# Shamir-Lab/Faucet

Measured on AMD Instinct MI355X. Metric: canonical k-mers/s (load+scan) at k=31, 100bp reads; % HBM roofline, higher is better.
Workload: dtype u64

## Files before the change

### faucet_amd/build.py

```python
from __future__ import annotations

import glob
import os
import subprocess
import sys

HERE = os.path.dirname(os.path.abspath(__file__))
ROOT = os.path.dirname(HERE)
CSRC = os.path.join(HERE, "csrc")
LIB = os.path.join(HERE, "libfaucet_gpu.so")
CLI = os.path.join(HERE, "faucet")
HIP_SOURCES = ["api.hip", "pack.hip", "load.hip", "load_slices.hip", "estimate.hip", "scan_pure.hip", "scan_walk.hip", "scan_table.hip", "scan_harvest.hip", "diag.hip", "text.hip", "stage3.hip", "stage3_emit.hip", "stage3_join.hip", "pairs.hip", "group.hip"]
CPP_SOURCES = ["sizing.cpp", "raw_plan.cpp", "tips_plan.cpp"]
HEADERS = ["fgpu_ctx.h", "fgpu_device.h", "fgpu_flags.h", "load_common.h", "walk_tables.h", "stage3_bits.h", "build_graph.h", os.path.join(ROOT, "include", "faucet_gpu.h")]
HIPCC = os.environ.get("HIPCC", "/opt/rocm/bin/hipcc")
FLAGS = ["-O3", "-std=c++17", "--offload-arch=gfx950", "-fPIC", "-Wall", "-Wno-unused-function", "-Wno-unused-result", "-Wno-unused-value"] + os.environ.get("FGPU_EXTRA_CXXFLAGS", "").split()


def _newer(target, deps):
    if not os.path.exists(target):
        return True
    t = os.path.getmtime(target)
    return any(os.path.getmtime(d) > t for d in deps)


def _run(cmd):
    r = subprocess.run(cmd, capture_output=True, text=True)
    if r.returncode != 0:
        sys.stderr.write(" ".join(cmd) + "\n" + r.stdout + r.stderr)
        raise RuntimeError("build failed: " + os.path.basename(cmd[-1]))
    if r.stderr.strip():
        sys.stderr.write(r.stderr)


def build(force: bool = False, jobs: int = 6) -> str:
    objdir = os.path.join(HERE, "build")
    os.makedirs(objdir, exist_ok=True)
    hdrs = [h if os.path.isabs(h) else os.path.join(CSRC, h) for h in HEADERS]
    objs, procs = [], []
    for src in HIP_SOURCES + CPP_SOURCES:
        sp = os.path.join(CSRC, src)
        obj = os.path.join(objdir, src + ".o")
        objs.append(obj)
        if force or _newer(obj, [sp] + hdrs):
            cmd = [HIPCC] + FLAGS + (["-x", "hip"] if src.endswith(".hip") else []) + ["-c", sp, "-o", obj]
            procs.append((cmd, subprocess.Popen(cmd, stdout=subprocess.PIPE, stderr=subprocess.STDOUT, text=True)))
            if len(procs) >= jobs:
# ... 28 lines not shown
```

### faucet_amd/csrc/fgpu_ctx.h

```cpp
#pragma once
#include <chrono>
#include <hip/hip_runtime.h>
#include <stdint.h>
#include <stdio.h>
#include <string.h>

#include <string>
#include <thread>
#include <vector>

#include "../../include/faucet_gpu.h"
#include <deque>

#include "fgpu_device.h"

#define FGPU_PADW 8
#define FGPU_USUAL_SPAN (1ULL << 26)
#define FGPU_MAX_SPAN (1ULL << 26)

#define FGPU_RANGE_EVENTS 16
#define FGPU_RANGE_MIN (1ULL << 20)

struct DevBuf {
    void*    p = nullptr;
// ... 486 lines not shown
int fgpu_stage_pack(fgpu_ctx* ctx, const fgpu_reads* reads);
int fgpu_stage_pack_block(fgpu_ctx* ctx, const fgpu_reads* reads, PackedBlock** out);
int fgpu_packed_acquire(fgpu_ctx* ctx, uint64_t T, uint64_t n_reads, int state, const char* who, PackedBlock** out, uint64_t beside = 0);
int fgpu_offs_keep(fgpu_ctx* ctx, void* dst, const uint64_t* src, uint64_t n);
int fgpu_offs_check_report(fgpu_ctx* ctx);
int fgpu_packed_digest(fgpu_ctx* ctx, const PackedBlock* b, bool verify);
int fgpu_host_batch_done(fgpu_ctx* ctx, const fgpu_reads* reads);
int fgpu_stage_load(fgpu_ctx* ctx, const void* codes, const void* bad, uint64_t T, uint64_t n_words);
int fgpu_resident_keep(fgpu_ctx* ctx);
int fgpu_resident_adopt(fgpu_ctx* ctx, const PackedBlock& b, const fgpu_kept_reads* reads = nullptr);
void fgpu_adopted_release(fgpu_ctx* ctx, std::vector<void*>* blocks);
int fgpu_stage_pack_keep(fgpu_ctx* ctx, const fgpu_reads* reads, uint64_t budget_left, PackedBlock* out, bool* no_memory);
void fgpu_estimate_drop_kept(fgpu_ctx* ctx);
int fgpu_load_sweep(fgpu_ctx* ctx);
int fgpu_stage_fixup(fgpu_ctx* ctx, const uint32_t* prefix);
int fgpu_stage_presence(fgpu_ctx* ctx);
int fgpu_epoch_before_batch(fgpu_ctx* ctx, uint64_t span);
int fgpu_epoch_after_batch(fgpu_ctx* ctx, uint64_t span);
enum { FGPU_TAKE_OK = 0, FGPU_TAKE_NO_BUDGET, FGPU_TAKE_NO_MEMORY };
int fgpu_resident_take(fgpu_ctx* ctx, const uint64_t (&parts)[5], bool budgeted, ResidentBatch** out, uint64_t* total);
int fgpu_pull_counters(fgpu_ctx* ctx);
int fgpu_check_reads(fgpu_ctx* ctx, const fgpu_reads* r);
void fgpu_load_pass_policy(fgpu_ctx* ctx);
int fgpu_load_pass_counters(fgpu_ctx* ctx);
int fgpu_load_pass_end(fgpu_ctx* ctx, fgpu_load_stats* stats);
int fgpu_load_pair_begin(fgpu_ctx* ctx);
int fgpu_load_pair_end(fgpu_ctx* ctx);
void fgpu_resident_reset(fgpu_ctx* ctx, bool keep_going);
int fgpu_stage_scan_pure(fgpu_ctx* ctx, uint64_t* n_pieces, bool one_range);
bool fgpu_walk_no_overlap();
int fgpu_stage_scan_walk(fgpu_ctx* ctx, uint64_t n_pieces);
int fgpu_stage_scan_need(fgpu_ctx* ctx);
int fgpu_stage_scan_need_lookup(fgpu_ctx* ctx, uint64_t w_lo, uint64_t w_hi);
int fgpu_stage_scan_need_prewalk(fgpu_ctx* ctx, uint64_t w_lo, uint64_t w_hi);
int fgpu_scan_refresh_planes(fgpu_ctx* ctx, BatchBufs* b);
int fgpu_scan_build_cand(fgpu_ctx* ctx, BatchBufs* b);
int fgpu_scan_import_probe(fgpu_ctx* ctx, const void* dev_entries, uint64_t n, uint64_t after_seq, uint32_t* dfilter, uint64_t dfilter_bits,
                           uint64_t* max_seq, uint64_t* n_newer, uint64_t digest[2]);
int fgpu_stage_scan_debug_drop(fgpu_ctx* ctx, uint64_t w_lo, uint64_t w_hi);
int fgpu_estimate_range_counts(fgpu_ctx* ctx, uint64_t g0, uint64_t g1, uint64_t h[2 * FGPU_EST_LEVELS + 1]);
void fgpu_estimate_close(fgpu_ctx* ctx, void** later);
int fgpu_estimate_finish(fgpu_ctx* ctx, fgpu_estimate* e, const char* who);
int fgpu_util_count_segments(fgpu_ctx* ctx, const void* bad, uint64_t n_words, int minlen);
int fgpu_util_popcount(fgpu_ctx* ctx, const void* dev, uint64_t nbytes, unsigned long long* dev_out);
int fgpu_util_or(fgpu_ctx* ctx, void* dst, const void* src, uint64_t nbytes);
int fgpu_util_probe_hash(fgpu_ctx* ctx, const uint64_t* d_kmers, uint64_t n, uint64_t* d_canon, uint64_t* d_hA, uint64_t* d_hB);
int fgpu_util_probe_contains(fgpu_ctx* ctx, const uint32_t* bloom, const uint64_t* d_canon, uint64_t n, unsigned char* d_out);
int fgpu_util_probe_stage3(fgpu_ctx* ctx, const uint64_t* d_kmers, uint64_t n, int mode, signed char* d_out);
int fgpu_scan_alloc(fgpu_ctx* ctx);
int fgpu_scan_harvest(fgpu_ctx* ctx, BatchBufs* b);
int fgpu_long_pairs_batch(fgpu_ctx* ctx, const fgpu_stop* d_stops, uint64_t n_stops, uint64_t n_reads);
int fgpu_long_pairs_reset(fgpu_ctx* ctx);
int fgpu_long_pairs_close(fgpu_ctx* ctx);
int fgpu_place_pair(fgpu_ctx* ctx);
int fgpu_scan_reset(fgpu_ctx* ctx);
int fgpu_scan_grow(fgpu_ctx* ctx, uint64_t new_cap);
int fgpu_scan_reserve(fgpu_ctx* ctx, uint64_t records);
int fgpu_scan_clear_table(fgpu_ctx* ctx);
int fgpu_scan_dump_order_impl(fgpu_ctx* ctx, const uint64_t* d_keys, const uint64_t* counts, const uint64_t* buckets, uint64_t n_phases, uint64_t n, uint32_t* order_host);
int fgpu_scan_regrow_empty(fgpu_ctx* ctx, uint64_t new_cap);
```

### faucet_amd/csrc/fgpu_device.h

```cpp
#pragma once
#include <hip/hip_runtime.h>
#include <stdint.h>

#define FD_SEED0 0xffaa54ffe6e6e6e7ULL
#define FD_SEED1 0x1140aada557088a4ULL

struct FdParams {
    int      k;
    int      j;
    int      n_hash;
    int      max_spacer;
    uint64_t kmask;
    uint64_t tai_mask;
};

__device__ __forceinline__ uint64_t fd_revcomp(uint64_t x, int k) {
    uint64_t y = __builtin_bitreverse64(x ^ 0xAAAAAAAAAAAAAAAAULL);
    y = ((y >> 1) & 0x5555555555555555ULL) | ((y & 0x5555555555555555ULL) << 1);
    return y >> (64 - 2 * k);
}

__device__ __forceinline__ uint64_t fd_canon(uint64_t x, int k) {
    uint64_t r = fd_revcomp(x, k);
    return x < r ? x : r;
// ... 61 lines not shown
__device__ __forceinline__ bool fd_bloom_contains_canon_lazy(const uint32_t* __restrict__ bloom, uint64_t canon,
                                                             uint64_t tai_mask, int n_hash) {
    const uint64_t hA = fd_old_hash(canon, FD_SEED0) & tai_mask;
    if (!((bloom[hA >> 5] >> (hA & 31)) & 1u)) return false;
    if (n_hash == 1) return true;
    const uint64_t hB = fd_old_hash(canon, FD_SEED1) & tai_mask;
    uint64_t h = (hA + hB) & tai_mask;
    for (int i = 1; i < n_hash; i++) {
        if (!((bloom[h >> 5] >> (h & 31)) & 1u)) return false;
        h = (h + hB) & tai_mask;
    }
    return true;
}

__device__ __forceinline__ void fd_bloom_set(uint32_t* bloom, uint64_t hA, uint64_t hB, uint64_t tai_mask, int n_hash) {
    uint64_t h = hA;
    for (int i = 0; i < n_hash; i++) {
        uint32_t bit = 1u << (h & 31);
        if (!(bloom[h >> 5] & bit)) atomicOr(&bloom[h >> 5], bit);
        h = (h + hB) & tai_mask;
    }
}

__device__ __forceinline__ uint64_t fd_mix(uint64_t x) {
    x ^= x >> 33;
    x *= 0xff51afd7ed558ccdULL;
    x ^= x >> 33;
    x *= 0xc4ceb9fe1a85ec53ULL;
    x ^= x >> 33;
    return x;
}

__device__ __forceinline__ int fd_lane() { return (int)(threadIdx.x & 63); }

__device__ __forceinline__ void wave_add(unsigned long long* dst, unsigned long long v) {
    for (int o = 32; o > 0; o >>= 1) v += __shfl_down(v, o, 64);
    if (fd_lane() == 0 && v) atomicAdd(dst, v);
}

__device__ __forceinline__ void block_add(unsigned long long* dst, unsigned long long v) {
    __shared__ unsigned long long part[4];
    for (int o = 32; o > 0; o >>= 1) v += __shfl_down(v, o, 64);
    if (fd_lane() == 0) part[threadIdx.x >> 6] = v;
    __syncthreads();
    if (threadIdx.x == 0) {
        const unsigned long long t = part[0] + part[1] + part[2] + part[3];
        if (t) atomicAdd(dst, t);
    }
    __syncthreads();
}
```

### faucet_amd/csrc/scan_pure.hip

```cpp
#include <algorithm>

#include "fgpu_ctx.h"
#include "fgpu_flags.h"

namespace {

__global__ void __launch_bounds__(256) k_scan_same(const uint64_t* __restrict__ codes, const uint64_t* __restrict__ kept_codes, uint64_t n_code_words,
                                                   const uint64_t* __restrict__ bad, const uint64_t* __restrict__ kept_bad, uint64_t n_words,
                                                   uint32_t* same) {
    bool differ = false;
    for (uint64_t i = (uint64_t)blockIdx.x * blockDim.x + threadIdx.x; i < n_code_words; i += (uint64_t)gridDim.x * blockDim.x) {
        differ |= codes[i] != kept_codes[i];
        if (i < n_words) differ |= bad[i] != kept_bad[i];
    }
    if (__ballot(differ) && fd_lane() == 0) *same = 0;
}

__global__ void __launch_bounds__(256) k_scan_valid(const uint64_t* __restrict__ codes, const uint64_t* __restrict__ bad,
                                                    uint64_t T, uint64_t n_words, FdParams fp, const uint32_t* __restrict__ bloom,
                                                    const uint64_t* __restrict__ sure, const uint32_t* __restrict__ same,
                                                    uint64_t* __restrict__ valid, DevCounters* cnt) {
    unsigned long long n_ok = 0, n_reused = 0;
    const uint64_t total = n_words * 64;
    const bool reuse = sure && *same != 0;
    for (uint64_t p = (uint64_t)blockIdx.x * blockDim.x + threadIdx.x; p < total; p += (uint64_t)gridDim.x * blockDim.x) {
        bool ok = p < T && fd_window_ok(bad, p, fp.k);
        bool v = false;
        if (ok) {
            n_ok++;
            if (reuse && ((sure[p >> 6] >> (p & 63)) & 1ULL)) {
                v = true;
                n_reused++;
            } else {
                v = fd_bloom_contains_canon(bloom, fd_canon(fd_kmer_at(codes, p, fp.k), fp.k), fp.tai_mask, fp.n_hash);
            }
        }
        uint64_t vm = __ballot(v);
        if (fd_lane() == 0) valid[p >> 6] = vm;
    }
    block_add(&cnt->kmers, n_ok);
    block_add(&cnt->valid_reused, n_reused);
}

__global__ void __launch_bounds__(256) k_scan_pieces(const uint64_t* __restrict__ valid, const uint64_t* __restrict__ bad,
                                                     uint64_t n_words, FdParams fp, int check_segment,
                                                     unsigned long long* pm, uint64_t* __restrict__ ps, DevCounters* cnt) {
    unsigned long long n_pieces = 0;
    for (uint64_t w = (uint64_t)blockIdx.x * blockDim.x + threadIdx.x; w < n_words; w += (uint64_t)gridDim.x * blockDim.x) {
        uint64_t vw = valid[w];
        uint64_t prev = w ? valid[w - 1] >> 63 : 0;
        uint64_t starts = vw & ~((vw << 1) | prev);
// ... 118 lines not shown
    while (lo < hi) {
        const uint64_t mid = (lo + hi + 1) >> 1;
        if ((offs[mid] - off0) + mid <= s0) lo = mid; else hi = mid - 1;
    }
    piece_read[i] = (uint32_t)lo;
}

__global__ void __launch_bounds__(256) k_scan_flags(const uint64_t* __restrict__ codes, const uint64_t* __restrict__ pm,
                                                    const uint64_t* __restrict__ need, uint64_t T, uint64_t w_lo, uint64_t w_hi, FdParams fp, const uint32_t* __restrict__ bloom,
                                                    unsigned long long* ff, unsigned long long* fb, unsigned long long* cf0,
                                                    unsigned long long* cf1, unsigned long long* cb0, unsigned long long* cb1,
                                                    DevCounters* cnt) {
    const int lane = fd_lane();
    const uint64_t n_waves = ((uint64_t)gridDim.x * blockDim.x) >> 6;
    const uint64_t n_chunks = (w_hi - w_lo + 3) / 4;
    unsigned long long n_eval = 0, n_piece = 0;
    for (uint64_t chunk = ((uint64_t)blockIdx.x * blockDim.x + threadIdx.x) >> 6; chunk < n_chunks; chunk += n_waves) {
        uint64_t mine = 0;
        if (lane < 8) {
            const uint64_t w = w_lo + chunk * 4 + (lane & 3);
            if (w < w_hi) {
                const uint64_t tmask = (w + 1) * 64 <= T ? ~0ULL : (T > w * 64 ? (1ULL << (T - w * 64)) - 1 : 0ULL);
                const uint64_t pmw = pm[w] & tmask, nd = need[w] & tmask;
                if (lane < 4) {
                    mine = nd & pmw & ((pmw >> 1) | (pm[w + 1] << 63));
                    n_eval += __popcll(nd);
                    n_piece += __popcll(pmw);
                } else {
                    mine = nd & pmw & ((pmw << 1) | (w ? pm[w - 1] >> 63 : 0ULL));
                }
            }
        }
        uint64_t m[8];
        int cum[9];
        cum[0] = 0;
#pragma unroll
        for (int q = 0; q < 8; q++) {
            m[q] = __shfl(mine, q, 64);
            cum[q + 1] = cum[q] + __popcll(m[q]);
        }
        for (int t = lane; t < cum[8]; t += 64) {
            int q = 0;
            uint64_t mq = m[0];
            int before = 0;
#pragma unroll
            for (int c = 1; c < 8; c++)
                if (t >= cum[c]) { q = c; mq = m[c]; before = cum[c]; }
            const int bit = select_bit(mq, t - before);
            const uint64_t w = w_lo + chunk * 4 + (q & 3);
            const uint64_t pos = w * 64 + bit;
            const uint64_t km = fd_kmer_at(codes, pos, fp.k);
            bool flag;
            int njc;
            const unsigned long long bm = 1ULL << bit;
            if (q < 4) {
                test_for_junction(km, fd_base_at(codes, pos + fp.k), fp, bloom, flag, njc);
                if (flag) atomicOr(&ff[w], bm);
                if (njc & 1) atomicOr(&cf0[w], bm);
                if (njc & 2) atomicOr(&cf1[w], bm);
            } else {
                test_for_junction(fd_revcomp(km, fp.k), fd_base_at(codes, pos - 1) ^ 2, fp, bloom, flag, njc);
                if (flag) atomicOr(&fb[w], bm);
                if (njc & 1) atomicOr(&cb0[w], bm);
                if (njc & 2) atomicOr(&cb1[w], bm);
            }
        }
    }
    block_add(&cnt->flag_positions, n_eval);
    block_add(&cnt->piece_positions, n_piece);
}

struct FlagPool {
    unsigned long long mf[64], mb[64];
    int excl[64];
};

struct FlagChain {
    uint64_t key;
    uint64_t hA, hB;
    uint32_t w;
    uint32_t st;
// ... 281 lines not shown
    BatchBufs& bb = *ctx->cur;
    *n_pieces = 0;
    bb.n_pieces = 0;
    bb.n_ranges = 0;
    if (bb.T == 0) return FGPU_OK;
    const uint64_t wb = (bb.n_words + FGPU_PADW) * 8;
    int rc;
    DevBuf* planes[] = {&bb.valid, &bb.pm, &bb.ps, &bb.ff, &bb.fb, &bb.cf0, &bb.cf1, &bb.cb0, &bb.cb1, &bb.inF, &bb.inB, &bb.lk, &bb.nF, &bb.nB, &bb.need};
    for (DevBuf* b : planes)
        if ((rc = fgpu_ensure_b(ctx, b, wb))) return rc;
    if ((rc = fgpu_ensure_b(ctx, &bb.ps_prefix, (bb.n_words + FGPU_PADW + bb.n_words / SCAN_BLOCK + 2) * 4))) return rc;
    const double t_a = fgpu_host_now();
    FGPU_HIP(hipMemsetAsync(bb.valid.p, 0, wb, ctx->stream));
    FGPU_HIP(hipMemsetAsync(bb.pm.p, 0, wb, ctx->stream));
    FGPU_HIP(hipMemsetAsync(bb.ps.p, 0, wb, ctx->stream));

    const unsigned grid = fgpu_grid(bb.n_words * 64, 256);
    const unsigned wgrid = fgpu_grid(bb.n_words, 256);
    if ((rc = fgpu_util_count_segments(ctx, ctx->cur->bad.p, ctx->cur->n_words, ctx->fd.k + 2 * ctx->fd.j + 1))) return rc;
    const uint64_t kept_index = ctx->scan_resident_base + ctx->scan_batch_index;
    const ResidentBatch* kept = kept_index < ctx->resident_count ? ctx->resident[kept_index] : nullptr;
    ctx->scan_batch_index++;
    if (kept && (kept->T != bb.T || kept->n_words != bb.n_words)) kept = nullptr;
    const bool taken = ctx->scan_take_kept != nullptr;
    if (taken) kept = ctx->scan_take_kept;
    if (kept) {
        if ((rc = fgpu_ensure_b(ctx, &bb.same, 64))) return rc;
        FGPU_HIP(hipMemsetAsync(bb.same.p, 0x01, 4, ctx->stream));
        const uint64_t ncw = 2 * bb.n_words;
        if (!taken)
            FGPU_LAUNCH("scan_same", k_scan_same, fgpu_grid(ncw, 256), 256, (const uint64_t*)bb.codes.p, (const uint64_t*)kept->codes_p(), ncw,
                        (const uint64_t*)bb.bad.p, (const uint64_t*)kept->bad_p(), bb.n_words, (uint32_t*)bb.same.p);
    }
    FGPU_LAUNCH("scan_valid", k_scan_valid, grid, 256, (const uint64_t*)bb.codes.p, (const uint64_t*)bb.bad.p, bb.T, bb.n_words, ctx->fd,
                (const uint32_t*)ctx->bloo2, kept ? (const uint64_t*)kept->sure.p : (const uint64_t*)nullptr,
                kept ? (const uint32_t*)bb.same.p : (const uint32_t*)nullptr, (uint64_t*)bb.valid.p, ctx->counters);
    const int check_segment = ctx->fd.k < 2 * ctx->fd.j + 2;
    FGPU_LAUNCH("scan_pieces", k_scan_pieces, wgrid, 256, (const uint64_t*)bb.valid.p, (const uint64_t*)bb.bad.p, bb.n_words, ctx->fd,
                check_segment, (unsigned long long*)bb.pm.p, (uint64_t*)bb.ps.p, ctx->counters);
    uint32_t* prefix = (uint32_t*)bb.ps_prefix.p;
    uint32_t* block_sums = prefix + bb.n_words + FGPU_PADW;
    const uint32_t nblk = fgpu_blocks(bb.n_words + 1, SCAN_BLOCK);
    const uint64_t nw1 = bb.n_words + 1;
    FGPU_LAUNCH("prefix_block", k_prefix_block, nblk, SCAN_BLOCK, (const uint64_t*)bb.ps.p, nw1, prefix, block_sums);
    FGPU_LAUNCH("prefix_sums", k_prefix_sums, 1, SCAN_BLOCK, block_sums, nblk);
    FGPU_LAUNCH("prefix_apply", k_prefix_apply, fgpu_blocks(nw1, 256), 256, prefix, (const uint32_t*)block_sums, nw1);
    FGPU_HIP(hipMemcpyAsync(ctx->counters_host, ctx->counters, sizeof(DevCounters), hipMemcpyDeviceToHost, ctx->stream));
    const double t_b = fgpu_host_now();
    FGPU_HIP(fgpu_sync_stream(ctx, ctx->stream));
    const double t_c = fgpu_host_now();
    ctx->host_ms[2] += t_b - t_a;
    ctx->host_ms[3] += t_c - t_b;
    bb.max_piece_span = ctx->counters_host->max_read_len + 64;
    const uint64_t np = ctx->counters_host->pieces - ctx->scan_pieces_seen;
    ctx->scan_pieces_seen = ctx->counters_host->pieces;
    *n_pieces = np;
    bb.n_pieces = np;
    if ((rc = fgpu_ensure_b(ctx, &bb.pieces, (np + 1) * sizeof(uint2)))) return rc;
    if (np) {
        FGPU_LAUNCH("piece_list", k_scan_piece_list, wgrid, 256, (const uint64_t*)bb.ps.p, (const uint64_t*)bb.pm.p,
                    (const uint32_t*)prefix, bb.n_words, (uint2*)bb.pieces.p);
        if (ctx->record_stops) {
            if ((rc = fgpu_ensure_b(ctx, &bb.piece_read, np * 4))) return rc;
            FGPU_LAUNCH("piece_read", k_scan_piece_read, fgpu_blocks(np, 256), 256, (const uint2*)bb.pieces.p, np, bb.d_offs, bb.n_reads,
                        (uint32_t*)bb.piece_read.p);
        }
        if ((rc = fgpu_stage_scan_need(ctx))) return rc;
        DevBuf* outs[] = {&bb.ff, &bb.fb, &bb.cf0, &bb.cf1, &bb.cb0, &bb.cb1};
        for (DevBuf* o : outs) FGPU_HIP(hipMemsetAsync(o->p, 0, wb, ctx->stream));
// ... 6 lines not shown
```

### faucet_amd/csrc/scan_walk.hip

```cpp
#include <cstring>
#include <algorithm>

#include "fgpu_flags.h"
#include "walk_tables.h"

namespace {

__device__ __forceinline__ uint32_t uf_find(uint32_t* parent, uint32_t x) {
    uint32_t p = ld_agent(&parent[x]);
    while (p != x) {
        uint32_t gp = ld_agent(&parent[p]);
        if (gp != p) atomicMin(&parent[x], gp);
        x = p;
        p = gp;
    }
    return x;
}

__device__ __forceinline__ void uf_union(uint32_t* parent, uint32_t a, uint32_t b) {
    for (;;) {
        a = uf_find(parent, a);
        b = uf_find(parent, b);
        if (a == b) return;
        if (a < b) { uint32_t t = a; a = b; b = t; }
        uint32_t old = atomicCAS(&parent[a], a, b);
        if (old == a) return;
    }
}

constexpr int W_OWNER_BITS = 24;
constexpr uint64_t W_OWNER_MASK = (1ULL << W_OWNER_BITS) - 1;
constexpr uint64_t W_EPOCH_MASK = 0xFFULL << 56;
constexpr uint32_t W_NO_OWNER = (uint32_t)W_OWNER_MASK;
__device__ __forceinline__ uint32_t wt_filter_bit(const WTable& wt, uint32_t h32) { return (h32 * 0x85EBCA6Bu) >> wt.fshift; }

__device__ __forceinline__ void wt_register(const WTable& wt, uint32_t* parent, uint32_t h32, uint32_t piece, DevCounters* cnt) {
// ... 75 lines not shown
    const WinDesc wd = make_window(pl, lo, hi);
    if (blockIdx.x < word_blocks) {
        const uint64_t w = (wd.lo >> 6) + (uint64_t)blockIdx.x * blockDim.x + threadIdx.x;
        if (w * 64 >= pos_end) return;
        unsigned long long m = pl.pm[w] & (pl.inF[w] | pl.inB[w] | pl.ff[w] | pl.fb[w]);
        if (w == (wd.lo >> 6)) m &= ~0ULL << (wd.lo & 63);
        if ((w + 1) * 64 > pos_end) m &= (1ULL << (pos_end & 63)) - 1;
        while (m) {
            const int b = __builtin_ctzll(m);
            m &= m - 1;
            const uint64_t p = w * 64 + (uint64_t)b;
            uint32_t li;
            uint2 pc;
            if (piece_in_window(pl, wd, p, li, pc)) wt_register(wt, parent, pl.kh[p], li, cnt);
        }
    } else if (blockIdx.x < word_blocks + piece_blocks) {
        const uint32_t li = (blockIdx.x - word_blocks) * blockDim.x + threadIdx.x;
        if (li >= wd.n) return;
        const uint2 pc = pl.pieces[wd.first_piece + li];
        const uint32_t len = pc.y + (uint32_t)fp.k - 1;
        wt_register(wt, parent, pl.kh[pc.x + (len / 2 - (uint32_t)fp.k / 2)], li, cnt);
        for (uint32_t q = (uint32_t)fp.max_spacer - 1; q < pc.y; q++) wt_register(wt, parent, pl.kh[pc.x + q], li, cnt);
    } else {
        const uint64_t t = (uint64_t)(blockIdx.x - word_blocks - piece_blocks) * blockDim.x + threadIdx.x;
        const uint64_t stride = (uint64_t)(gridDim.x - word_blocks - piece_blocks) * blockDim.x;
        for (int r = 0; r < FGPU_DELTA_RING; r++) {
            if (!ds.list[r]) continue;
            const uint64_t n = *ds.count[r];
            for (uint64_t i = t; i < n; i += stride) wt_register(wt, nullptr, ds.list[r][i], W_NO_OWNER, cnt);
        }
    }
}

__global__ void __launch_bounds__(256) k_walk_link(Planes pl, FdParams fp, WTable wt, uint32_t* parent, uint64_t lo, uint64_t hi,
                                                   uint64_t pos_end, uint32_t* roots_state) {
    const WinDesc wd = make_window(pl, lo, hi);
    if (roots_state && blockIdx.x == 0 && threadIdx.x == 0) { roots_state[0] = 0; roots_state[1] = 0; }
    const uint64_t base0 = wd.lo & ~63ULL;
    constexpr int U = 4;
    for (uint64_t base = base0 + (uint64_t)blockIdx.x * (256 * U); base < pos_end; base += (uint64_t)gridDim.x * (256 * U)) {
        uint64_t p[U];
        uint32_t h[U], fw[U];
        bool act[U];
#pragma unroll
        for (int u = 0; u < U; u++) {
            p[u] = base + (uint64_t)u * 256 + threadIdx.x;
            act[u] = p[u] >= wd.lo && p[u] < pos_end && ((pl.pm[p[u] >> 6] >> (p[u] & 63)) & 1ULL);
        }
#pragma unroll
        for (int u = 0; u < U; u++) h[u] = act[u] ? pl.kh[p[u]] : 0u;
#pragma unroll
        for (int u = 0; u < U; u++) {
            const uint32_t b = wt_filter_bit(wt, h[u]);
            fw[u] = act[u] ? ((wt.bits[b >> 5] >> (b & 31)) & 1u) : 0u;
        }
#pragma unroll
        for (int u = 0; u < U; u++) {
            bool hit = false;
            if (fw[u]) {
                uint64_t slot = 0;
                uint32_t owner = wt_owner(wt, h[u], slot);
                if (owner != U_INF) {
                    uint32_t li;
                    uint2 pc;
                    if (piece_in_window(pl, wd, p[u], li, pc)) {
                        hit = true;
                        if (owner == W_NO_OWNER) {
// ... 2075 lines not shown
    WTable wt;
    uint32_t *roots_state, *root_list;
};

struct LargeClusterRule {
    uint32_t ko_heavy;
    uint32_t ko_heavy_w;
    int ovw_rounds;
    bool ovw_on;
};

constexpr int OVW_MARK_LOG2 = 22;

template <class FullPass>
static int walk_dbg_compare(fgpu_ctx* ctx, hipStream_t st, const uint64_t* plane0, const uint64_t* plane1, uint64_t n_words, FullPass full, const char* what,
                            uint64_t batch, uint64_t lo) {
    uint64_t* scratch = nullptr;
    unsigned long long* out = nullptr;
    FGPU_HIP(hipMalloc(&scratch, 2 * n_words * 8));
    FGPU_HIP(hipMalloc(&out, 32));
    FGPU_HIP(hipMemsetAsync(out, 0, 32, st));
    FGPU_HIP(full(scratch));
    hipLaunchKernelGGL(k_dbg_diff, dim3(64), dim3(256), 0, st, (const uint64_t*)scratch, plane0, n_words, out, 0);
    if (plane1) hipLaunchKernelGGL(k_dbg_diff, dim3(64), dim3(256), 0, st, (const uint64_t*)(scratch + n_words), plane1, n_words, out, 1);
    unsigned long long h[4] = {0, 0, 0, 0};
    FGPU_HIP(hipMemcpyAsync(h, out, 32, hipMemcpyDeviceToHost, st));
    FGPU_HIP(hipStreamSynchronize(st));
    ctx->refresh_mismatch += h[0] + h[1];
    if (h[0] + h[1]) fprintf(stderr, "[fgpu] %s: %llu + %llu words differ, batch %llu window at %llu\n", what, h[0], h[1], (unsigned long long)batch, (unsigned long long)lo);
    (void)hipFree(scratch); (void)hipFree(out);
    return FGPU_OK;
}

static int walk_refresh_prepared(fgpu_ctx* ctx, BatchBufs& bb, const JTable& jt, hipStream_t walk_stream, bool* cand_ok) {
    *cand_ok = false;
    if (!(ctx->delta_ready && bb.planes_gen == ctx->hint_gen)) {
        FGPU_LAUNCH("walk_lookup", k_refresh_lookup, fgpu_grid(bb.n_words * 64, 256), 256, (const uint64_t*)bb.codes.p, (const uint64_t*)bb.pm.p, bb.n_words,
                    ctx->fd, jt, (const uint32_t*)jt.filter, jt.filter_mask, (uint64_t*)bb.nF.p, (uint64_t*)bb.nB.p, (const uint32_t*)bb.kh.p, 0, (uint64_t*)nullptr);
        ctx->refresh_full++;
        return FGPU_OK;
    }
    *cand_ok = !ctx->no_sparse_link && bb.cand.p && bb.cand_gen == ctx->hint_gen;
    if (ctx->delta_keys || ctx->refresh_delta)
        FGPU_LAUNCH("walk_lookup", k_refresh_lookup, fgpu_grid(bb.n_words * 64, 256), 256, (const uint64_t*)bb.codes.p, (const uint64_t*)bb.pm.p, bb.n_words,
                    ctx->fd, jt, (const uint32_t*)ctx->delta_filter.p, ctx->delta_filter_bits - 1, (uint64_t*)bb.nF.p, (uint64_t*)bb.nB.p,
                    (const uint32_t*)bb.kh.p, 1, *cand_ok ? (uint64_t*)bb.cand.p : (uint64_t*)nullptr);
    ctx->refresh_delta++;
    if (!ctx->dbg_delta_check) return FGPU_OK;
    const auto full = [&](uint64_t* scratch) {
        hipLaunchKernelGGL(k_refresh_lookup, dim3(fgpu_grid(bb.n_words * 64, 256)), dim3(256), 0, walk_stream, (const uint64_t*)bb.codes.p, (const uint64_t*)bb.pm.p,
                           bb.n_words, ctx->fd, jt, (const uint32_t*)jt.filter, jt.filter_mask, scratch, scratch + bb.n_words, (const uint32_t*)bb.kh.p, 0,
                           (uint64_t*)nullptr);
        return hipSuccess;
    };
    return walk_dbg_compare(ctx, walk_stream, (const uint64_t*)bb.nF.p, (const uint64_t*)bb.nB.p, bb.n_words, full, "merged in-map planes against planes made again",
                            bb.seq, 0);
}

static int walk_wait_range(fgpu_ctx* ctx, const WalkBatch& wb, uint64_t pos_end) {
    BatchBufs& bb = wb.bb;
    if (bb.n_ranges <= 1) return FGPU_OK;
    const uint64_t last = pos_end - 1;
    const uint64_t r = last < bb.range_first ? 0 : std::min<uint64_t>(1 + (last - bb.range_first) / bb.range_span, bb.n_ranges - 1);
    if (r < bb.ranges_waited) return FGPU_OK;
    FGPU_HIP(hipStreamWaitEvent(wb.walk_stream, bb.range_ev[r % FGPU_RANGE_EVENTS], 0));
    bb.ranges_waited = r + 1;
// ... 18 lines not shown

static int walk_register(fgpu_ctx* ctx, const WalkKnobs& kn, const WalkBatch& wb, const WalkWindow& w) {
    const BatchBufs& bb = wb.bb;
    DeltaSrc ds;
    memset(&ds, 0, sizeof(ds));
    const uint64_t delta_est = ctx->delta_ring_keys + (uint64_t)(3.0 * (double)bb.n_pieces * (double)w.lo / (double)wb.T);
    const bool refresh_window = !ctx->refresh_snapshot && delta_est > (w.pos_end - w.lo) / kn.refresh_div;
    if (refresh_window) {
        const uint64_t w_first = w.lo >> 6, w_last = std::min<uint64_t>(bb.n_words, (w.pos_end + 63) / 64);
        FGPU_LAUNCH("walk_lookup", k_need_lookup, fgpu_grid((w_last - w_first) * 64, 256), 256, (const uint64_t*)bb.codes.p, (const uint64_t*)bb.pm.p, w_last,
                    ctx->fd, wb.jt, (uint64_t*)bb.nF.p, (uint64_t*)bb.nB.p, (uint32_t*)bb.kh.p, w_first);
    } else {
        if (!ctx->refresh_snapshot)
            for (int r = 1; r < FGPU_DELTA_RING && (uint64_t)r <= ctx->delta_next; r++) {
                const DeltaList& dl = ctx->delta_ring[(ctx->delta_next - r) % FGPU_DELTA_RING];
                ds.list[r - 1] = (const uint32_t*)dl.list.p;
                ds.count[r - 1] = (const unsigned long long*)dl.count.p;
            }
        if (w.lo) {
            ds.list[FGPU_DELTA_RING - 1] = (const uint32_t*)wb.created->list.p;
            ds.count[FGPU_DELTA_RING - 1] = (const unsigned long long*)wb.created->count.p;
        }
    }
    const unsigned word_blocks = fgpu_blocks((w.pos_end - (w.lo & ~63ULL) + 63) / 64, 256);
    const unsigned piece_blocks = fgpu_blocks(w.max_pieces, 256);
    const unsigned delta_blocks = refresh_window ? 64u : (unsigned)std::min<uint64_t>(4096, std::max<uint64_t>(64, delta_est / kn.delta_per_block));
    FGPU_LAUNCH("walk_lookup", k_walk_register, word_blocks + piece_blocks + delta_blocks, 256, wb.pl, ctx->fd, w.wt, w.uf_parent, w.lo, w.hi, w.pos_end, ctx->counters,
                word_blocks, piece_blocks, ds);
    return FGPU_OK;
}

static int walk_link(fgpu_ctx* ctx, const WalkBatch& wb, const WalkWindow& w) {
    const BatchBufs& bb = wb.bb;
    const unsigned full_grid = std::min(fgpu_blocks(w.pos_end - (w.lo & ~63ULL), 1024), 4096u);
    if (!(wb.cand_ok && w.lo == 0)) {
        FGPU_LAUNCH("walk_link", k_walk_link, full_grid, 256, wb.pl, ctx->fd, w.wt, w.uf_parent, w.lo, w.hi, w.pos_end, w.roots_state);
        if (ctx->refresh_snapshot) ctx->full_links++;
        return FGPU_OK;
    }
    const uint64_t link_words = ((w.pos_end + 63) >> 6) - (w.lo >> 6);
    uint64_t* const lk = (uint64_t*)bb.lk.p + (w.lo >> 6);
    FGPU_LAUNCH("walk_link", k_walk_link_sparse, std::min(fgpu_blocks(link_words, 256), 4096u), 256, wb.pl, ctx->fd, w.wt, w.uf_parent, w.lo, w.hi, w.pos_end,
                w.roots_state, (const uint64_t*)bb.cand.p, (uint64_t*)bb.lk.p);
    ctx->sparse_links++;
    if (!ctx->dbg_delta_check) return FGPU_OK;
    const auto full = [&](uint64_t* scratch) {
        const hipError_t e = hipMemcpyAsync(scratch, lk, link_words * 8, hipMemcpyDeviceToDevice, wb.walk_stream);
        hipLaunchKernelGGL(k_walk_link, dim3(full_grid), dim3(256), 0, wb.walk_stream, wb.pl, ctx->fd, w.wt, w.uf_parent, w.lo, w.hi, w.pos_end, (uint32_t*)nullptr);
        return e;
    };
    return walk_dbg_compare(ctx, wb.walk_stream, (const uint64_t*)lk, (const uint64_t*)nullptr, link_words, full, "sparse link pass: lk plane against the full pass's",
                            bb.seq, w.lo);
}

static LargeClusterRule large_cluster_rule(fgpu_ctx* ctx, const WalkKnobs& kn) {
    const DevCounters& seen = *ctx->counters_host;
    LargeClusterRule r;
    r.ko_heavy = (!ctx->walk_ko || !(ctx->walk_ko_always || seen.max_cluster >= ctx->walk_ko)) ? 0u : ctx->walk_ko;
    const bool repeats_seen = seen.walk_parallel * 50 > seen.walked_pieces ||
                              (ctx->walk_ko_always && seen.walked_pieces < (1ULL << 17) && ctx->delta_next >= 2 && ctx->repeats_seen_before);
    if (repeats_seen) ctx->repeats_seen_before = true;
    const uint32_t ko_total = std::min<uint32_t>(ctx->walk_ko_weight, 0xFFFFu);
    const uint32_t ko_avg = kn.ko_avg >= 0 ? (uint32_t)kn.ko_avg : repeats_seen ? 8u : 12u;
    const uint32_t ko_total_rep = kn.ko_avg_min > 0 ? (uint32_t)kn.ko_avg_min : repeats_seen ? 16u : std::min<uint32_t>(255u, 3 * ko_total / 8);
    r.ko_heavy_w = (r.ko_heavy && ko_total) ? (ko_total | (ko_avg << 16) | (ko_total_rep << 24)) : 0u;
    r.ovw_rounds = !r.ko_heavy ? 0 : std::min(ctx->ovw_rounds, OVW_MAX_ROUNDS);
    const bool ovw_seen_enough = seen.walked_pieces >= (1ULL << 17);
    r.ovw_on = r.ovw_rounds > 0 && ((ctx->walk_ko_always && (ctx->delta_next < 2 || !ovw_seen_enough)) || seen.walk_parallel * 256 > seen.walked_pieces);
    return r;
}

static int walk_large_tables(fgpu_ctx* ctx, const WalkBatch& wb, const LargeClusterRule& rule, KoTables& kt, OvwTables& ot) {
    kt.hk_key = ctx->ko_hk;
    kt.hk_head = ctx->ko_hk + ctx->ko_hk_cap;
    kt.hk_turn = ctx->ko_hk + 2 * (size_t)ctx->ko_hk_cap;
    kt.hk_mask = ctx->ko_hk_cap - 1;
    kt.occ_id = (uint64_t*)ctx->ko_occ;
    kt.occ_entry = (uint32_t*)(kt.occ_id + ctx->ko_occ_cap);
    kt.occ_rank = kt.occ_entry + ctx->ko_occ_cap;
    kt.occ_next = kt.occ_rank + ctx->ko_occ_cap;
    kt.occ_cap = ctx->ko_occ_cap;
    kt.trace = nullptr;
#ifdef FGPU_KO_TRACE
    if (!ctx->ko_trace.p) {
        if (int trc = fgpu_ensure(ctx, &ctx->ko_trace, ((1ULL << 23) + 4096 * 1024) * 8)) return trc;
// ... 258 lines not shown
```

Measured before the change: 6.079 billion.

## Compact sparse bloom and table probes across wave lanes in scan and link kernels

```diff
diff --git a/faucet_amd/build.py b/faucet_amd/build.py
--- a/faucet_amd/build.py
+++ b/faucet_amd/build.py
@@ -12,7 +12,7 @@
 CLI = os.path.join(HERE, "faucet")
 HIP_SOURCES = ["api.hip", "pack.hip", "load.hip", "load_slices.hip", "estimate.hip", "scan_pure.hip", "scan_walk.hip", "scan_table.hip", "scan_harvest.hip", "diag.hip", "text.hip", "stage3.hip", "stage3_emit.hip", "stage3_join.hip", "pairs.hip", "group.hip"]
 CPP_SOURCES = ["sizing.cpp", "raw_plan.cpp", "tips_plan.cpp"]
-HEADERS = ["fgpu_ctx.h", "fgpu_device.h", "fgpu_flags.h", "load_common.h", "walk_tables.h", "stage3_bits.h", "build_graph.h", os.path.join(ROOT, "include", "faucet_gpu.h")]
+HEADERS = ["fgpu_ctx.h", "fgpu_device.h", "fgpu_flags.h", "dense_hits.h", "load_common.h", "walk_tables.h", "stage3_bits.h", "build_graph.h", os.path.join(ROOT, "include", "faucet_gpu.h")]
 HIPCC = os.environ.get("HIPCC", "/opt/rocm/bin/hipcc")
 FLAGS = ["-O3", "-std=c++17", "--offload-arch=gfx950", "-fPIC", "-Wall", "-Wno-unused-function", "-Wno-unused-result", "-Wno-unused-value"] + os.environ.get("FGPU_EXTRA_CXXFLAGS", "").split()
 
diff --git a/faucet_amd/csrc/dense_hits.h b/faucet_amd/csrc/dense_hits.h
--- /dev/null
+++ b/faucet_amd/csrc/dense_hits.h
@@ -0,0 +1,58 @@
+#pragma once
+#include "fgpu_flags.h"
+
+namespace {
+
+template <int U>
+struct DenseItems {
+    uint64_t m[U];
+    int cum[U + 1];
+    __device__ __forceinline__ explicit DenseItems(const uint64_t (&masks)[U]) {
+        cum[0] = 0;
+#pragma unroll
+        for (int u = 0; u < U; u++) {
+            m[u] = masks[u];
+            cum[u + 1] = cum[u] + __popcll(masks[u]);
+        }
+    }
+    __device__ __forceinline__ int total() const { return cum[U]; }
+    __device__ __forceinline__ void item(int t, int& q, int& bit) const {
+        q = 0;
+        uint64_t mq = m[0];
+        int before = 0;
+#pragma unroll
+        for (int c = 1; c < U; c++)
+            if (t >= cum[c]) { q = c; mq = m[c]; before = cum[c]; }
+        bit = select_bit(mq, t - before);
+    }
+};
+
+template <int U>
+struct DenseBits {
+    uint64_t r[U];
+    __device__ __forceinline__ DenseBits() {
+#pragma unroll
+        for (int c = 0; c < U; c++) r[c] = 0;
+    }
+    __device__ __forceinline__ void put(int round, uint64_t ballot) {
+#pragma unroll
+        for (int c = 0; c < U; c++)
+            if (c == round) r[c] = ballot;
+    }
+    __device__ __forceinline__ uint64_t word(const DenseItems<U>& it, int u) const {
+        const int r0 = it.cum[u] >> 6, s = it.cum[u] & 63;
+        uint64_t lo = 0, hi = 0;
+#pragma unroll
+        for (int c = 0; c < U; c++) {
+            if (c == r0) lo = r[c];
+            if (c == r0 + 1) hi = r[c];
+        }
+        const uint64_t packed = (lo >> s) | ((hi << 1) << (63 - s));
+        const int lane = fd_lane();
+        const uint64_t mu = it.m[u];
+        const bool mine = ((mu >> lane) & 1ULL) && ((packed >> __popcll(mu & ((1ULL << lane) - 1))) & 1ULL);
+        return __ballot(mine);
+    }
+};
+
+}
diff --git a/faucet_amd/csrc/fgpu_ctx.h b/faucet_amd/csrc/fgpu_ctx.h
--- a/faucet_amd/csrc/fgpu_ctx.h
+++ b/faucet_amd/csrc/fgpu_ctx.h
@@ -542,6 +542,7 @@
 int fgpu_stage_scan_walk(fgpu_ctx* ctx, uint64_t n_pieces);
 int fgpu_stage_scan_need(fgpu_ctx* ctx);
 int fgpu_stage_scan_need_lookup(fgpu_ctx* ctx, uint64_t w_lo, uint64_t w_hi);
+int fgpu_dbg_compare_planes(fgpu_ctx* ctx, hipStream_t st, const uint64_t* scratch, const uint64_t* plane, uint64_t n_words, const char* what, uint64_t batch);
 int fgpu_stage_scan_need_prewalk(fgpu_ctx* ctx, uint64_t w_lo, uint64_t w_hi);
 int fgpu_scan_refresh_planes(fgpu_ctx* ctx, BatchBufs* b);
 int fgpu_scan_build_cand(fgpu_ctx* ctx, BatchBufs* b);
diff --git a/faucet_amd/csrc/fgpu_device.h b/faucet_amd/csrc/fgpu_device.h
--- a/faucet_amd/csrc/fgpu_device.h
+++ b/faucet_amd/csrc/fgpu_device.h
@@ -117,6 +117,7 @@
 }
 
 __device__ __forceinline__ int fd_lane() { return (int)(threadIdx.x & 63); }
+__device__ __forceinline__ uint32_t fd_wave() { return (uint32_t)__builtin_amdgcn_readfirstlane((int)(threadIdx.x >> 6)); }
 
 __device__ __forceinline__ void wave_add(unsigned long long* dst, unsigned long long v) {
     for (int o = 32; o > 0; o >>= 1) v += __shfl_down(v, o, 64);
diff --git a/faucet_amd/csrc/scan_pure.hip b/faucet_amd/csrc/scan_pure.hip
--- a/faucet_amd/csrc/scan_pure.hip
+++ b/faucet_amd/csrc/scan_pure.hip
@@ -1,7 +1,7 @@
 #include <algorithm>
 
 #include "fgpu_ctx.h"
-#include "fgpu_flags.h"
+#include "dense_hits.h"
 
 namespace {
 
@@ -17,6 +17,51 @@
 }
 
 __global__ void __launch_bounds__(256) k_scan_valid(const uint64_t* __restrict__ codes, const uint64_t* __restrict__ bad,
+                                                    uint64_t T, uint64_t n_words, FdParams fp, const uint32_t* __restrict__ bloom,
+                                                    const uint64_t* __restrict__ sure, const uint32_t* __restrict__ same,
+                                                    uint64_t* __restrict__ valid, DevCounters* cnt) {
+    constexpr int U = 8;
+    unsigned long long n_ok = 0, n_reused = 0;
+    const int lane = fd_lane();
+    const bool reuse = sure && *same != 0;
+    const uint64_t n_waves = ((uint64_t)gridDim.x * blockDim.x) >> 6;
+    const uint64_t n_chunks = (n_words + U - 1) / U;
+    for (uint64_t chunk = (uint64_t)blockIdx.x * (blockDim.x >> 6) + fd_wave(); chunk < n_chunks; chunk += n_waves) {
+        const uint64_t w0 = chunk * U;
+        uint64_t known[U], items[U];
+#pragma unroll
+        for (int u = 0; u < U; u++) {
+            const uint64_t p = (w0 + u) * 64 + lane;
+            const bool ok = w0 + u < n_words && p < T && fd_window_ok(bad, p, fp.k);
+            const uint64_t okm = __ballot(ok);
+            known[u] = reuse && w0 + u < n_words ? okm & sure[w0 + u] : 0ULL;
+            items[u] = okm & ~known[u];
+            if (lane == 0) { n_ok += __popcll(okm); n_reused += __popcll(known[u]); }
+        }
+        const DenseItems<U> it(items);
+        DenseBits<U> probed;
+        for (int r = 0; r * 64 < it.total(); r++) {
+            const int t = r * 64 + lane;
+            bool v = false;
+            if (t < it.total()) {
+                int q, bit;
+                it.item(t, q, bit);
+                const uint64_t p = (w0 + (uint64_t)q) * 64 + (uint64_t)bit;
+                v = fd_bloom_contains_canon(bloom, fd_canon(fd_kmer_at(codes, p, fp.k), fp.k), fp.tai_mask, fp.n_hash);
+            }
+            probed.put(r, __ballot(v));
+        }
+#pragma unroll
+        for (int u = 0; u < U; u++) {
+            const uint64_t vm = known[u] | probed.word(it, u);
+            if (lane == 0 && w0 + u < n_words) valid[w0 + u] = vm;
+        }
+    }
+    block_add(&cnt->kmers, n_ok);
+    block_add(&cnt->valid_reused, n_reused);
+}
+
+__global__ void __launch_bounds__(256) k_scan_valid_lane(const uint64_t* __restrict__ codes, const uint64_t* __restrict__ bad,
                                                     uint64_t T, uint64_t n_words, FdParams fp, const uint32_t* __restrict__ bloom,
                                                     const uint64_t* __restrict__ sure, const uint32_t* __restrict__ same,
                                                     uint64_t* __restrict__ valid, DevCounters* cnt) {
@@ -201,21 +246,12 @@
             }
         }
         uint64_t m[8];
-        int cum[9];
-        cum[0] = 0;
-#pragma unroll
-        for (int q = 0; q < 8; q++) {
-            m[q] = __shfl(mine, q, 64);
-            cum[q + 1] = cum[q] + __popcll(m[q]);
-        }
-        for (int t = lane; t < cum[8]; t += 64) {
-            int q = 0;
-            uint64_t mq = m[0];
-            int before = 0;
-#pragma unroll
-            for (int c = 1; c < 8; c++)
-                if (t >= cum[c]) { q = c; mq = m[c]; before = cum[c]; }
-            const int bit = select_bit(mq, t - before);
+#pragma unroll
+        for (int q = 0; q < 8; q++) m[q] = __shfl(mine, q, 64);
+        const DenseItems<8> it(m);
+        for (int t = lane; t < it.total(); t += 64) {
+            int q, bit;
+            it.item(t, q, bit);
             const uint64_t w = w_lo + chunk * 4 + (q & 3);
             const uint64_t pos = w * 64 + bit;
             const uint64_t km = fd_kmer_at(codes, pos, fp.k);
@@ -563,9 +599,30 @@
             FGPU_LAUNCH("scan_same", k_scan_same, fgpu_grid(ncw, 256), 256, (const uint64_t*)bb.codes.p, (const uint64_t*)kept->codes_p(), ncw,
                         (const uint64_t*)bb.bad.p, (const uint64_t*)kept->bad_p(), bb.n_words, (uint32_t*)bb.same.p);
     }
+    DevCounters dbg_before;
+    if (ctx->dbg_delta_check) FGPU_HIP(hipMemcpyAsync(&dbg_before, ctx->counters, sizeof(DevCounters), hipMemcpyDeviceToHost, ctx->stream));
     FGPU_LAUNCH("scan_valid", k_scan_valid, grid, 256, (const uint64_t*)bb.codes.p, (const uint64_t*)bb.bad.p, bb.T, bb.n_words, ctx->fd,
                 (const uint32_t*)ctx->bloo2, kept ? (const uint64_t*)kept->sure.p : (const uint64_t*)nullptr,
                 kept ? (const uint32_t*)bb.same.p : (const uint32_t*)nullptr, (uint64_t*)bb.valid.p, ctx->counters);
+    if (ctx->dbg_delta_check) {
+        uint64_t* scratch = nullptr;
+        FGPU_HIP(hipMalloc(&scratch, bb.n_words * 8 + sizeof(DevCounters)));
+        DevCounters* scnt = (DevCounters*)(scratch + bb.n_words);
+        FGPU_HIP(hipMemsetAsync(scnt, 0, sizeof(DevCounters), ctx->stream));
+        hipLaunchKernelGGL(k_scan_valid_lane, dim3(grid), dim3(256), 0, ctx->stream, (const uint64_t*)bb.codes.p, (const uint64_t*)bb.bad.p, bb.T, bb.n_words, ctx->fd,
+                           (const uint32_t*)ctx->bloo2, kept ? (const uint64_t*)kept->sure.p : (const uint64_t*)nullptr,
+                           kept ? (const uint32_t*)bb.same.p : (const uint32_t*)nullptr, scratch, scnt);
+        DevCounters now, lane_form;
+        FGPU_HIP(hipMemcpyAsync(&now, ctx->counters, sizeof(DevCounters), hipMemcpyDeviceToHost, ctx->stream));
+        FGPU_HIP(hipMemcpyAsync(&lane_form, scnt, sizeof(DevCounters), hipMemcpyDeviceToHost, ctx->stream));
+        rc = fgpu_dbg_compare_planes(ctx, ctx->stream, scratch, (const uint64_t*)bb.valid.p, bb.n_words, "dense validity pass: valid plane against the per-lane pass's", bb.seq);
+        (void)hipFree(scratch);
+        if (rc) return rc;
+        if (now.kmers - dbg_before.kmers != lane_form.kmers || now.valid_reused - dbg_before.valid_reused != lane_form.valid_reused) {
+            ctx->refresh_mismatch++;
+            fprintf(stderr, "[fgpu] dense validity pass: counters differ from the per-lane pass's, batch %llu\n", (unsigned long long)bb.seq);
+        }
+    }
     const int check_segment = ctx->fd.k < 2 * ctx->fd.j + 2;
     FGPU_LAUNCH("scan_pieces", k_scan_pieces, wgrid, 256, (const uint64_t*)bb.valid.p, (const uint64_t*)bb.bad.p, bb.n_words, ctx->fd,
                 check_segment, (unsigned long long*)bb.pm.p, (uint64_t*)bb.ps.p, ctx->counters);
diff --git a/faucet_amd/csrc/scan_walk.hip b/faucet_amd/csrc/scan_walk.hip
--- a/faucet_amd/csrc/scan_walk.hip
+++ b/faucet_amd/csrc/scan_walk.hip
@@ -1,7 +1,7 @@
 #include <cstring>
 #include <algorithm>
 
-#include "fgpu_flags.h"
+#include "dense_hits.h"
 #include "walk_tables.h"
 
 namespace {
@@ -143,7 +143,86 @@
     }
 }
 
+__device__ __forceinline__ uint32_t wt_owner_unfiltered(const WTable& wt, uint32_t h32, uint64_t& slot) {
+    uint64_t s = (uint64_t)h32 & wt.mask;
+    for (uint64_t n = 0; n <= wt.mask; n++) {
+        const uint64_t w = wt.keys[s];
+        if ((w & W_EPOCH_MASK) != wt.epoch) return U_INF;
+        if ((uint32_t)(w >> W_OWNER_BITS) == h32) { slot = s; return (uint32_t)(w & W_OWNER_MASK); }
+        s = (s + 1) & wt.mask;
+    }
+    return U_INF;
+}
+
+constexpr int LINK_U = 4;
 __global__ void __launch_bounds__(256) k_walk_link(Planes pl, FdParams fp, WTable wt, uint32_t* parent, uint64_t lo, uint64_t hi,
+                                                   uint64_t pos_end, uint32_t* roots_state) {
+    constexpr int U = LINK_U;
+    const WinDesc wd = make_window(pl, lo, hi);
+    if (roots_state && blockIdx.x == 0 && threadIdx.x == 0) { roots_state[0] = 0; roots_state[1] = 0; }
+    const int lane = fd_lane();
+    const uint64_t base0 = wd.lo & ~63ULL, lk_end = (pos_end + 63) & ~63ULL;
+    for (uint64_t base = base0 + (uint64_t)blockIdx.x * (256 * U); base < pos_end; base += (uint64_t)gridDim.x * (256 * U)) {
+        const uint64_t wave_base = base + 64 * fd_wave();
+        uint32_t h[U];
+        bool act[U];
+        uint64_t fm[U];
+#pragma unroll
+        for (int u = 0; u < U; u++) {
+            const uint64_t p = wave_base + (uint64_t)u * 256 + lane;
+            act[u] = p >= wd.lo && p < pos_end && ((pl.pm[p >> 6] >> (p & 63)) & 1ULL);
+        }
+#pragma unroll
+        for (int u = 0; u < U; u++) h[u] = act[u] ? pl.kh[wave_base + (uint64_t)u * 256 + lane] : 0u;
+#pragma unroll
+        for (int u = 0; u < U; u++) {
+            const uint32_t b = wt_filter_bit(wt, h[u]);
+            const bool f = act[u] && ((wt.bits[b >> 5] >> (b & 31)) & 1u);
+            fm[u] = __ballot(f);
+        }
+        const DenseItems<U> it(fm);
+        DenseBits<U> hits;
+        for (int r = 0; r * 64 < it.total(); r++) {
+            const int t = r * 64 + lane;
+            const bool have = t < it.total();
+            int q = 0, bit = 0;
+            if (have) it.item(t, q, bit);
+            uint32_t hq = 0;
+#pragma unroll
+            for (int u = 0; u < U; u++) {
+                const uint32_t v = (uint32_t)__shfl((int)h[u], bit, 64);
+                if (q == u) hq = v;
+            }
+            bool hit = false;
+            if (have) {
+                const uint64_t p = wave_base + (uint64_t)q * 256 + (uint64_t)bit;
+                uint64_t slot = 0;
+                uint32_t owner = wt_owner_unfiltered(wt, hq, slot);
+                if (owner != U_INF) {
+                    uint32_t li;
+                    uint2 pc;
+                    if (piece_in_window(pl, wd, p, li, pc)) {
+                        hit = true;
+                        if (owner == W_NO_OWNER) {
+                            const unsigned long long mine = (unsigned long long)(wt.epoch | ((uint64_t)hq << W_OWNER_BITS) | (uint64_t)li);
+                            owner = (uint32_t)(atomicMin((unsigned long long*)&wt.keys[slot], mine) & W_OWNER_MASK);
+                        }
+                        if (owner != li && owner != W_NO_OWNER) uf_union(parent, li, owner);
+                    }
+                }
+            }
+            hits.put(r, __ballot(hit));
+        }
+#pragma unroll
+        for (int u = 0; u < U; u++) {
+            const uint64_t m = hits.word(it, u);
+            const uint64_t pw = wave_base + (uint64_t)u * 256;
+            if (lane == 0 && pw < lk_end) pl.lk[pw >> 6] = m;
+        }
+    }
+}
+
+__global__ void __launch_bounds__(256) k_walk_link_lane(Planes pl, FdParams fp, WTable wt, uint32_t* parent, uint64_t lo, uint64_t hi,
                                                    uint64_t pos_end, uint32_t* roots_state) {
     const WinDesc wd = make_window(pl, lo, hi);
     if (roots_state && blockIdx.x == 0 && threadIdx.x == 0) { roots_state[0] = 0; roots_state[1] = 0; }
@@ -2285,6 +2364,20 @@
     return FGPU_OK;
 }
 
+int fgpu_dbg_compare_planes(fgpu_ctx* ctx, hipStream_t st, const uint64_t* scratch, const uint64_t* plane, uint64_t n_words, const char* what, uint64_t batch) {
+    unsigned long long* out = nullptr;
+    FGPU_HIP(hipMalloc(&out, 32));
+    FGPU_HIP(hipMemsetAsync(out, 0, 32, st));
+    hipLaunchKernelGGL(k_dbg_diff, dim3(64), dim3(256), 0, st, scratch, plane, n_words, out, 0);
+    unsigned long long h[4] = {0, 0, 0, 0};
+    FGPU_HIP(hipMemcpyAsync(h, out, 32, hipMemcpyDeviceToHost, st));
+    FGPU_HIP(hipStreamSynchronize(st));
+    ctx->refresh_mismatch += h[0];
+    if (h[0]) fprintf(stderr, "[fgpu] %s: %llu words differ, batch %llu\n", what, h[0], (unsigned long long)batch);
+    (void)hipFree(out);
+    return FGPU_OK;
+}
+
 static int walk_refresh_prepared(fgpu_ctx* ctx, BatchBufs& bb, const JTable& jt, hipStream_t walk_stream, bool* cand_ok) {
     *cand_ok = false;
     if (!(ctx->delta_ready && bb.planes_gen == ctx->hint_gen)) {
@@ -2369,25 +2462,28 @@
 
 static int walk_link(fgpu_ctx* ctx, const WalkBatch& wb, const WalkWindow& w) {
     const BatchBufs& bb = wb.bb;
-    const unsigned full_grid = std::min(fgpu_blocks(w.pos_end - (w.lo & ~63ULL), 1024), 4096u);
+    const unsigned full_grid = std::min(fgpu_blocks(w.pos_end - (w.lo & ~63ULL), 256 * LINK_U), 4096u);
+    const unsigned lane_grid = std::min(fgpu_blocks(w.pos_end - (w.lo & ~63ULL), 1024), 4096u);
+    const uint64_t link_words = ((w.pos_end + 63) >> 6) - (w.lo >> 6);
+    uint64_t* const lk = (uint64_t*)bb.lk.p + (w.lo >> 6);
+    const char* what;
     if (!(wb.cand_ok && w.lo == 0)) {
         FGPU_LAUNCH("walk_link", k_walk_link, full_grid, 256, wb.pl, ctx->fd, w.wt, w.uf_parent, w.lo, w.hi, w.pos_end, w.roots_state);
         if (ctx->refresh_snapshot) ctx->full_links++;
-        return FGPU_OK;
-    }
-    const uint64_t link_words = ((w.pos_end + 63) >> 6) - (w.lo >> 6);
-    uint64_t* const lk = (uint64_t*)bb.lk.p + (w.lo >> 6);
-    FGPU_LAUNCH("walk_link", k_walk_link_sparse, std::min(fgpu_blocks(link_words, 256), 4096u), 256, wb.pl, ctx->fd, w.wt, w.uf_parent, w.lo, w.hi, w.pos_end,
-                w.roots_state, (const uint64_t*)bb.cand.p, (uint64_t*)bb.lk.p);
-    ctx->sparse_links++;
+        what = "dense link pass: lk plane against the per-lane pass's";
+    } else {
+        FGPU_LAUNCH("walk_link", k_walk_link_sparse, std::min(fgpu_blocks(link_words, 256), 4096u), 256, wb.pl, ctx->fd, w.wt, w.uf_parent, w.lo, w.hi, w.pos_end,
+                    w.roots_state, (const uint64_t*)bb.cand.p, (uint64_t*)bb.lk.p);
+        ctx->sparse_links++;
+        what = "sparse link pass: lk plane against the full pass's";
+    }
     if (!ctx->dbg_delta_check) return FGPU_OK;
     const auto full = [&](uint64_t* scratch) {
         const hipError_t e = hipMemcpyAsync(scratch, lk, link_words * 8, hipMemcpyDeviceToDevice, wb.walk_stream);
-        hipLaunchKernelGGL(k_walk_link, dim3(full_grid), dim3(256), 0, wb.walk_stream, wb.pl, ctx->fd, w.wt, w.uf_parent, w.lo, w.hi, w.pos_end, (uint32_t*)nullptr);
+        hipLaunchKernelGGL(k_walk_link_lane, dim3(lane_grid), dim3(256), 0, wb.walk_stream, wb.pl, ctx->fd, w.wt, w.uf_parent, w.lo, w.hi, w.pos_end, (uint32_t*)nullptr);
         return e;
     };
-    return walk_dbg_compare(ctx, wb.walk_stream, (const uint64_t*)lk, (const uint64_t*)nullptr, link_words, full, "sparse link pass: lk plane against the full pass's",
-                            bb.seq, w.lo);
+    return walk_dbg_compare(ctx, wb.walk_stream, (const uint64_t*)lk, (const uint64_t*)nullptr, link_words, full, what, bb.seq, w.lo);
 }
 
 static LargeClusterRule large_cluster_rule(fgpu_ctx* ctx, const WalkKnobs& kn) {
```

New measurement: 6.152 billion, median of 6. 1.2% higher.
